# DIAGNijmegen/bodyct-dram-emph-subtype

Hardware: AMD Instinct MI355X
Metric: CT volumes/sec (train step, 1x128x256x256) (higher is better)
Workload: dtype f32; 1 GPU; BASELINE configs[1]: resnet18segcls train step (fwd+loss+bwd+Adam), batch 2/GPU, 1x128x256x256, fp32, inputs resident in HBM; global_batch=2, parallelism=dp1, hip_graph=False, streams=2

## Files before the change

### bodyct-dram-emph-subtype_amd/csrc/bn.hip

```cpp
#include <stdlib.h>
#include <atomic>
#include "common.h"

namespace {

template <typename T>
__global__ void reduce_partials_kernel(const T* __restrict__ partial, double* __restrict__ out, int nparts,
                                       int RC, double tail, int has_tail) {
  __shared__ double sm[256];
  const int col = blockIdx.x * 64 + (threadIdx.x & 63);
  const int lane4 = threadIdx.x >> 6;
  const int S = gridDim.y, sidx = blockIdx.y;
  double s = 0.0;
  if (col < RC)
    for (int p = sidx + S * lane4; p < nparts; p += 4 * S) s += (double)partial[(long)p * RC + col];
  sm[threadIdx.x] = s;
  __syncthreads();
  if (lane4 == 0 && col < RC)
    out[(long)sidx * RC + col] = sm[threadIdx.x] + sm[threadIdx.x + 64] + sm[threadIdx.x + 128] + sm[threadIdx.x + 192];
  if (has_tail && blockIdx.x == 0 && blockIdx.y == 0 && threadIdx.x == 0) out[RC] = tail;
}

__global__ void bn_finalize_kernel(const double* __restrict__ sums, double count_host,
                                   const double* __restrict__ count_dev, const float* __restrict__ gamma,
// ... 20 lines not shown
  }
  const double is = 1.0 / sqrt(v + (double)eps);
  const float sc = (float)((double)gamma[c] * is);
  mean[c] = (float)m;
  invstd[c] = (float)is;
  scale[c] = sc;
  shift[c] = (float)((double)beta[c] - m * (double)gamma[c] * is);
}

struct FoldFinalize {
  double count;
  const float* gamma; const float* beta; float* rmean; float* rvar;
  float momentum, eps; int update;
  float* mean; float* invstd; float* scale; float* shift;
};
constexpr int FOLD_XMAX = 512;

__global__ __launch_bounds__(1024) void fold_partials_kernel(const float* __restrict__ partial, double* scratch,
                                                             double* __restrict__ sums, float* __restrict__ sums_f32,
                                                             float* __restrict__ f32_row1, const int nparts, const int RC,
                                                             const double tail,
                                                             const int has_tail, unsigned* __restrict__ ticket,
                                                             const FoldFinalize ff) {
  __shared__ double sm[1024];
  __shared__ double tot[64];
  __shared__ unsigned s_ticket;
  const int t64 = threadIdx.x & 63, lane4 = threadIdx.x >> 6;
  const int C = RC >> 1;
  const int col = ff.gamma ? (t64 >> 5) * C + blockIdx.x * 32 + (t64 & 31) : blockIdx.x * 64 + t64;
  const bool live = ff.gamma ? (blockIdx.x * 32 + (t64 & 31) < C) : (col < RC);
  const int S = gridDim.y, sidx = blockIdx.y;
// ... 12 lines not shown
  }
  sm[threadIdx.x] = s;
  __syncthreads();
  double total = 0.0;
  if (lane4 == 0) {
#pragma unroll
    for (int j = 0; j < 16; ++j) total += sm[t64 + 64 * j];
  }
  if (S > 1) {
    if (lane4 == 0 && live) scratch[(long)sidx * RC + col] = total;
    __threadfence();
    __syncthreads();
    if (threadIdx.x == 0) s_ticket = atomicAdd(&ticket[blockIdx.x], 1u);
    __syncthreads();
    if (s_ticket != (unsigned)S - 1) return;
    __threadfence();
    if (lane4 == 0 && live) {
      total = 0.0;
      int k = 0;
      for (; k + 8 <= S; k += 8) {
        double v[8];
#pragma unroll
        for (int j = 0; j < 8; ++j)
          v[j] = __hip_atomic_load(scratch + (long)(k + j) * RC + col, __ATOMIC_RELAXED, __HIP_MEMORY_SCOPE_AGENT);
#pragma unroll
        for (int j = 0; j < 8; ++j) total += v[j];
      }
      for (; k < S; ++k)
        total += __hip_atomic_load(scratch + (long)k * RC + col, __ATOMIC_RELAXED, __HIP_MEMORY_SCOPE_AGENT);
    }
// ... 436 lines not shown
    DRAM_LAUNCH_CHECK();
    hipLaunchKernelGGL((reduce_partials_kernel<double>), dim3((RC + 63) / 64, 1), dim3(256), 0, st,
                       (const double*)scratch, sums, S, RC, tail, has_tail);
  }
  DRAM_LAUNCH_CHECK();
  return DRAM_OK;
}

extern "C" int dram_fold_partials_stages(int nparts) {
  if (nparts <= 1024) return 1;
  const int s = (nparts + 511) / 512;
  return s > 64 ? 64 : s;
}

static int fold_launch(const float* partial, double* sums, double* scratch, float* sums_f32, float* f32_row1, int nparts,
                       int RC, double tail, int has_tail, const FoldFinalize& ff, hipStream_t st) {
  const int S = dram_fold_partials_stages(nparts);
  const int gx = ff.gamma ? (RC / 2 + 31) / 32 : (RC + 63) / 64;
  if (S > 1 && gx > FOLD_XMAX) return DRAM_ERR_UNSUPPORTED;
  unsigned* ticket = nullptr;
  if (S > 1) {
    ticket = reinterpret_cast<unsigned*>(scratch + (long)S * RC);
    const hipError_t e = hipMemsetAsync(ticket, 0, sizeof(unsigned) * gx, st);
    if (e != hipSuccess) return (int)e;
  }
  DramProf prof(DRAM_FAM_BN, 0, 0.0, 4.0 * (double)nparts * RC + 8.0 * RC, st);
  hipLaunchKernelGGL(fold_partials_kernel, dim3(gx, S), dim3(1024), 0, st, partial, scratch, sums, sums_f32, f32_row1,
                     nparts, RC, tail, has_tail, ticket, ff);
  DRAM_LAUNCH_CHECK();
  return DRAM_OK;
}

extern "C" int dram_fold_partials(const float* partial, double* sums, double* scratch, float* sums_f32, float* f32_row1,
                                  int nparts, int R, int C, double tail, int has_tail, dram_stream_t stream) {
  if (!partial || !sums || !scratch || nparts < 1 || R < 1 || C < 1) return DRAM_ERR_BAD_ARG;
  if (f32_row1 && (R != 2 || !sums_f32)) return DRAM_ERR_BAD_ARG;
  FoldFinalize ff{};
  return fold_launch(partial, sums, scratch, sums_f32, f32_row1, nparts, R * C, tail, has_tail, ff, (hipStream_t)stream);
}

extern "C" int dram_bn_fold_finalize(const float* partial, double* sums, double* scratch, int nparts, int C, double count,
                                     const float* gamma, const float* beta, float* running_mean, float* running_var,
                                     float momentum, float eps, int update_running, float* mean, float* invstd,
                                     float* scale, float* shift, dram_stream_t stream) {
  if (!partial || !sums || !scratch || nparts < 1 || C < 1 || count <= 0.0) return DRAM_ERR_BAD_ARG;
  if (!gamma || !beta || !mean || !invstd || !scale || !shift) return DRAM_ERR_BAD_ARG;
  if (update_running && (!running_mean || !running_var)) return DRAM_ERR_BAD_ARG;
  FoldFinalize ff{count, gamma, beta, running_mean, running_var, momentum, eps, update_running, mean, invstd, scale, shift};
  return fold_launch(partial, sums, scratch, nullptr, nullptr, nparts, 2 * C, 0.0, 0, ff, (hipStream_t)stream);
}

extern "C" int dram_bn_finalize(const double* sums, double count, const double* count_dev, const float* gamma,
                                const float* beta,
                                float* running_mean, float* running_var, float momentum, float eps,
                                int update_running, float* mean, float* invstd, float* scale, float* shift, int C,
                                dram_stream_t stream) {
  if (!gamma || !beta || !mean || !invstd || !scale || !shift || C < 1) return DRAM_ERR_BAD_ARG;
  if (!sums && (!running_mean || !running_var)) return DRAM_ERR_BAD_ARG;
  if (sums && !count_dev && count <= 0.0) return DRAM_ERR_BAD_ARG;
  if (update_running && (!running_mean || !running_var)) return DRAM_ERR_BAD_ARG;
  DramProf prof(DRAM_FAM_BN, 1, 0.0, 4.0 * 10.0 * C, (hipStream_t)stream);
  hipLaunchKernelGGL(bn_finalize_kernel, dim3((C + 255) / 256), dim3(256), 0, (hipStream_t)stream, sums, count,
                     count_dev, gamma, beta, running_mean, running_var, momentum, eps, update_running, mean, invstd, scale,
                     shift, C);
// ... 189 lines not shown
```

### bodyct-dram-emph-subtype_amd/csrc/head_loss.hip

```cpp
#include "common.h"

namespace {

template <int NOT, typename T>
__global__ __launch_bounds__(256) void head_fwd_kernel(const T* __restrict__ x, const float* __restrict__ w,
                                                       const float* __restrict__ bias, const float* __restrict__ lungs,
                                                       NearGeom ng, float* __restrict__ dense,
                                                       float* __restrict__ partial, int D, int H, int W, int NO,
                                                       int sigmoid, int nblk) {
  __shared__ float wl[NOT * 32 + NOT];
  __shared__ float red[4][NOT + 1];
  const int tid = threadIdx.x;
  for (int i = tid; i < NO * 32; i += 256) wl[i] = w[i];
  for (int i = tid; i < NO; i += 256) wl[NOT * 32 + i] = bias[i];
  __syncthreads();
  const long b = blockIdx.y;
  const long vps = (long)D * H * W;
  float acc[NOT + 1];
#pragma unroll
  for (int c = 0; c <= NOT; ++c) acc[c] = 0.f;
  for (long v = blockIdx.x * 256L + tid; v < vps; v += (long)gridDim.x * 256L) {
    asm volatile("" ::: "memory");
    float4 xv[8];
#pragma unroll
// ... 401 lines not shown
      !pse_bands || n_cle < 1 || n_pse < 1 || B < 1 || !out || !coef || !greg)
    return DRAM_ERR_BAD_ARG;
  RegTail a;
  a.partial = partial; a.nblk = nblk;
  a.reg[0] = reg_cle; a.reg[1] = reg_pse;
  a.label[0] = cle_labels; a.label[1] = pse_labels;
  a.weight[0] = cle_w; a.weight[1] = pse_w;
  a.bands[0] = cle_bands; a.bands[1] = pse_bands;
  a.nband[0] = n_cle; a.nband[1] = n_pse;
  a.B = B; a.N = voxels_total; a.smooth = smooth; a.beta = beta; a.gamma = gamma;
  a.out = out; a.coef = coef; a.greg = greg;
  hipLaunchKernelGGL(regloss_tail_kernel, dim3(1), dim3(256), 0, (hipStream_t)stream, a);
  DRAM_LAUNCH_CHECK();
  return DRAM_OK;
}
```

### bodyct-dram-emph-subtype_amd/engine.py

```python
from __future__ import annotations

import os
import time
from typing import Dict, List, Optional

import torch

from . import ops
from .ops import ConvGeom

Tensor = torch.Tensor

ARCHS = {
    "resnet18": ("basic", (2, 2, 2, 2)),
    "resnet34": ("basic", (3, 4, 6, 3)),
    "resnet50": ("bottleneck", (3, 4, 6, 3)),
}
EXPANSION = {"basic": 1, "bottleneck": 4}
STAGES = ((64, 1, 1), (128, 2, 1), (256, 1, 2), (512, 1, 4))
BN_EPS = 1e-5
BN_MOMENTUM = 0.1


class _State:
# ... 70 lines not shown
        bnp = c["bn"]
        scale, shift = st.eval_ss[bnp]
        zmask = c["z"] if c.get("ss") is None else None
        if st.dist is not None:
            self._flush_wgrad(st)
        if st.need_param:
            part = ops.bn_bwd_reduce(dz, zmask, c["y"], c["mean"], c["invstd"], True, scale, shift)
            _, sf = ops.reduce_partials(part, want_f32=True)
            st.grads[bnp + ".weight"] = sf[1]
            st.grads[bnp + ".bias"] = sf[0]
        y = c["y"] if zmask is None else None
        if c.get("b") and st.need_param:
            dy, colpart = ops.bn_bwd_apply_eval(dz, zmask, y, scale, shift, True, want_colsum=True)
            if colpart is None:
                colpart = ops.colsum(dy)
            st.grads[c["b"]] = ops.reduce_partials(colpart)[0].float()
            return dy
        return ops.bn_bwd_apply_eval(dz, zmask, y, scale, shift, True)

    def _bn_bwd(self, st: _State, c: dict, dz: Tensor) -> Tensor:
        if not st.training:
            return self._bn_bwd_eval(st, c, dz)
        bnp = c["bn"]
        zmask, (sc, sh) = (c["z"], (None, None)) if c.get("ss") is None else (None, c["ss"])
        part = c.pop("part", None)
        if part is None:
            part = ops.bn_bwd_reduce(dz, zmask, c["y"], c["mean"], c["invstd"], True, sc, sh)
        sums, sf = ops.reduce_partials(part, want_f32=True)
        st.grads[bnp + ".weight"] = sf[1]
        st.grads[bnp + ".bias"] = sf[0]
        count, count_dev = c["count"]
        if st.dist is not None and st.dist.sync_bn:
            work = st.dist.all_reduce_stats_async(sums)
            self._flush_wgrad(st)
            work.wait()
        if c.get("b"):
            dy, colpart = ops.bn_bwd_apply(dz, zmask, c["y"], c["mean"], c["invstd"], st.P[bnp + ".weight"], sums,
                                           count, True, sc, sh, want_colsum=True, count_dev=count_dev)
            if colpart is None:
                colpart = ops.colsum(dy)
            st.grads[c["b"]] = ops.reduce_partials(colpart)[0].float()
            return dy
        return ops.bn_bwd_apply(dz, zmask, c["y"], c["mean"], c["invstd"], st.P[bnp + ".weight"], sums, count,
                                True, sc, sh, count_dev=count_dev)

    def _conv_bn_fwd(self, st: _State, x, wname: str, bname: Optional[str], bnp: str, k: int, stride: int,
                     pad: int, dil: int, residual=None, rs: int = 1, xr=None, defer_z: bool = False):
        w = st.P[wname]
        pro = None
        split = None
        if isinstance(x, tuple):
            split = x
            x = None
            B, D, H, W, _ = split[0].shape
            Cin = split[0].shape[4] + split[1].shape[4]
        elif isinstance(x, dict):
# ... 327 lines not shown
        for li, ((planes, stride, dil), nblk) in enumerate(zip(STAGES, self.layers)):
            for bi in range(nblk):
                s = stride if bi == 0 else 1
                has_ds = bi == 0 and (stride != 1 or inplanes != planes * self.e)
                h, c = self._block_fwd(st, h, f"layer{li + 1}.{bi}", planes, s, dil, has_ds)
                block_ctx.append(c)
                inplanes = planes * self.e
            feats.append(h)
        x1, x4f = feats[0], feats[3]
        xup1, cu1 = self._up_fwd(st, x4f, x1, "us1")
        xup2, cu2 = self._up_fwd(st, xup1, xs, "us2")
        xup3, cu3 = self._conv_bn_fwd(st, xup2, "us3.0.weight", "us3.0.bias", "us3.1", 3, 1, 1, 1)

        n0, n1 = P["fcs.0.weight"].shape[0], P["fcs.1.weight"].shape[0]
        NO = n0 + n1
        hw = torch.cat([P["fcs.0.weight"].reshape(n0, 32), P["fcs.1.weight"].reshape(n1, 32)], 0).contiguous()
        hb = torch.cat([P["fcs.0.bias"], P["fcs.1.bias"]], 0).contiguous()
        sig = self.head == "reg"
        dense, partial = ops.head_fwd(xup3, hw, hb, lungs4 if sig else None, sig)
        sums = partial.sum(1)
        denom = sums[:, NO]
        if sig:
            outs = [sums[:, 0] / denom, sums[:, 1] / denom]
        else:
            pooled = sums[:, :NO] / denom[:, None]
            outs = [pooled[:, :n0].contiguous(), pooled[:, n0:].contiguous()]
        dense_list = [dense[:, :n0], dense[:, n0:]]
        saved = None
        if need_grad:
            saved = dict(st=st, x4=x4, y0=y0, xs=xs, mean0=mean0, invstd0=invstd0, count0=count0, ss0=ss0, amax=amax,
                         blocks=block_ctx, cu1=cu1, cu2=cu2, cu3=cu3, xup3=xup3, hw=hw, dense=dense, lungs4=lungs4,
                         denom=denom, n0=n0, n1=n1, xs_shape=tuple(xs.shape))
        elif keep_head:
            saved = dict(xup3=xup3, hw=hw, hb=hb, dense=dense, lungs4=lungs4, denom=denom, n0=n0, n1=n1)
        if need_grad:
            self._conv_lists[shape_key] = list(st.convs)
            st.packed.clear()
        if st.nbt:
            torch._foreach_add_(st.nbt, 1)
        return dense_list, outs, saved

    def _head_cotangents(self, saved, g_dense, g_outs):
        n0, n1 = saved["n0"], saved["n1"]
        NO = n0 + n1
        dense = saved["dense"]
        B = dense.shape[0]
        sig = self.head == "reg"
        dev = dense.device
        gpool = torch.zeros((B, NO), device=dev, dtype=torch.float32)
        denom = saved["denom"]
        if sig:
            if g_outs[0] is not None:
                gpool[:, 0] = g_outs[0] / denom
            if g_outs[1] is not None:
                gpool[:, 1] = g_outs[1] / denom
        else:
            if g_outs[0] is not None:
                gpool[:, :n0] = g_outs[0] / denom[:, None]
            if g_outs[1] is not None:
                gpool[:, n0:] = g_outs[1] / denom[:, None]
        gd = None
        if g_dense[0] is not None or g_dense[1] is not None:
            gd = torch.zeros_like(dense)
            if g_dense[0] is not None:
                gd[:, :n0] = g_dense[0]
            if g_dense[1] is not None:
                gd[:, n0:] = g_dense[1]
        return gpool, gd

    def _backward(self, saved, g_dense, g_outs):
        st: _State = saved["st"]
        dist = st.dist if st.need_param else None
        if dist is not None:
            dist.begin_backward(saved["dense"].device)
        if st.need_param and self._two_streams():
            st.side = ops.side_stream(saved["dense"].device.index)

        n0, n1 = saved["n0"], saved["n1"]
        NO = n0 + n1
        dense = saved["dense"]
        sig = self.head == "reg"
        gpool, gd = self._head_cotangents(saved, g_dense, g_outs)
        dxup3, wpart = ops.head_bwd(saved["xup3"], saved["hw"], dense if sig else None, gd, gpool,
                                    saved["lungs4"] if sig else None, sig)
        if st.need_param:
            wg = ops.reduce_partials(wpart.reshape(wpart.shape[0], 1, NO * 33)).reshape(NO, 33).float()
            st.grads["fcs.0.weight"] = wg[:n0, :32].reshape(n0, 32, 1, 1, 1).contiguous()
            st.grads["fcs.0.bias"] = wg[:n0, 32].contiguous()
            st.grads["fcs.1.weight"] = wg[n0:, :32].reshape(n1, 32, 1, 1, 1).contiguous()
            st.grads["fcs.1.bias"] = wg[n0:, 32].contiguous()
        if dist is not None:
            dist.grads_ready(st.grads, ["fcs.0.weight", "fcs.0.bias", "fcs.1.weight", "fcs.1.bias"])

        dxup2 = self._conv_bn_bwd(st, saved["cu3"], dxup3, nxt=saved["cu2"][1])
        dxup1, dskip_stem = self._up_bwd(st, saved["cu2"], dxup2, skip_view=True)
        d, dskip_x1 = self._up_bwd(st, saved["cu1"], dxup1)

        blocks = saved["blocks"]
        idx = len(blocks)
        for li in (3, 2, 1, 0):
            nblk = self.layers[li]
            for bi in reversed(range(nblk)):
                idx -= 1
                extra = dskip_x1 if (li == 1 and bi == 0) else None
                d = self._block_bwd(st, blocks[idx], d, extra_add=extra)
# ... 39 lines not shown
```

### bodyct-dram-emph-subtype_amd/med3d.py

```python
from __future__ import annotations

if not __package__:
    import _dropin
    __package__ = _dropin.adopt(__name__)

import os
from typing import List, Optional

import torch
import torch.nn as nn

from . import ops
from .engine import ARCHS, EXPANSION, Engine

__all__ = ["ResNetSegCls", "ResNetSegReg", "resnet18segcls", "resnet34segcls", "resnet50segcls",
           "resnet18segreg", "resnet34segreg", "resnet50segreg", "BasicBlock", "Bottleneck",
           "UpsampleConvBlock5d"]


def _conv3(cin, cout, stride=1, dilation=1):
    return nn.Conv3d(cin, cout, kernel_size=3, dilation=dilation, stride=stride, padding=dilation, bias=False)


class _Container(nn.Module):
# ... 53 lines not shown
                                                    need_x=need_x, need_param=need_param)
        ctx.saved_state = saved
        ctx.module = module
        return dense[0], dense[1], outs[0], outs[1]

    @staticmethod
    def backward(ctx, gd0, gd1, go0, go1):
        module = ctx.module
        saved, ctx.saved_state = ctx.saved_state, None
        if saved is None:
            raise RuntimeError("backward through the Med3D engine a second time (buffers were freed)")

        def c(t):
            return None if t is None else t.contiguous()

        grads = module._engine.backward(saved, [c(gd0), c(gd1)], [c(go0), c(go1)])
        out = [None, saved.get("dx") if ctx.needs_input_grad[1] else None, None]
        for name, p in module._named_tensors()[0]:
            out.append(grads.get(name) if p.requires_grad else None)
        return tuple(out)


class _ResNetSeg(nn.Module):
    HEAD = None

    def __init__(self, block, layers, shortcut_type="A", n_classes=(6, 3)):
        super().__init__()
        if shortcut_type != "A":
            raise NotImplementedError("only shortcut_type='A' (every reference conf) is implemented")
        self.inplanes = 64
        self.conv1 = nn.Conv3d(1, 64, kernel_size=7, stride=(2, 2, 2), padding=(3, 3, 3), bias=False)
# ... 227 lines not shown
```

### bodyct-dram-emph-subtype_amd/models.py

```python
from __future__ import annotations

if not __package__:
    import _dropin
    __package__ = _dropin.adopt(__name__)

import os
from types import SimpleNamespace
from typing import Dict, List, Optional

import numpy as np
import torch
import torch.nn as nn
import torch.nn.functional as F

from . import ops
from .optim import FusedAdam
from .utils import get_model_by_name

try:
    import pytorch_lightning as pl
    _Base = pl.LightningModule
except Exception:
    pl = None

# ... 124 lines not shown
def reg_train_loss(dense_outs, reg_outs, lungs, ems, cle_labels, pse_labels, cle_w, pse_w):
    B = dense_outs[0].shape[0]

    def vol(t):
        return t.reshape(B, *t.shape[-3:]).float().contiguous()

    def row(t, dtype=torch.float32):
        return t.reshape(B).to(dtype).contiguous()

    loss, lc, lp, mul, seg = _RegLossFn.apply(vol(dense_outs[0]), vol(dense_outs[1]), vol(lungs), vol(ems),
                                              row(reg_outs[0]), row(reg_outs[1]), row(cle_labels, torch.int64),
                                              row(pse_labels, torch.int64), row(cle_w), row(pse_w))
    return loss, dict(loss_cle=lc, loss_pse=lp, mul_loss=mul, seg_loss=seg)


def cls_train_loss(cls_outs, cle_labels, pse_labels, cle_cw, pse_cw):
    loss_cle = F.cross_entropy(cls_outs[0], cle_labels, weight=cle_cw)
    loss_pse = F.cross_entropy(cls_outs[1], pse_labels, weight=pse_cw)
    return loss_cle + loss_pse, dict(loss_cle=loss_cle, loss_pse=loss_pse)


def update_class_weights(weights: torch.Tensor, y_true: torch.Tensor, y_pred: torch.Tensor) -> torch.Tensor:
    labels = torch.unique(torch.cat([y_true, y_pred]))
    if labels.numel() != weights.numel():
        raise ValueError(f"class-weight update: {labels.numel()} classes occur, {weights.numel()} weights "
                         "(the reference's element-wise product fails the same way)")
    hit = (y_true[None, :] == labels[:, None])
    acc = (hit & (y_pred[None, :] == labels[:, None])).sum(1).double() / hit.sum(1).double()
    w = weights.double().to(acc.device) * (1.0 - acc)
    return (w / w.sum()).to(weights.dtype).cpu()

# ... 339 lines not shown
```

### bodyct-dram-emph-subtype_amd/ops.py

```python
from __future__ import annotations

import contextlib
import ctypes
import functools
import math
import os
import threading
import weakref
from dataclasses import dataclass
from typing import Dict, List, Optional, Tuple

import torch

from . import _lib
from ._lib import DramConvDesc

Tensor = torch.Tensor


def _L():
    return _lib.load()


_TLS = threading.local()
# ... 780 lines not shown
    B, D, H, W = (int(v) for v in in_shape)
    if min(B, D, H, W) < 1:
        raise ValueError(f"stem_bwd_data: bad input shape {tuple(in_shape)}")
    sfx = _act(dy, "dy", (B, stem_out(D), stem_out(H), stem_out(W), 64))
    _req(w, "w", shape=(64, 1, 7, 7, 7))
    nbytes = _L().dram_stem_bwd_data_workspace(B, D, H, W)
    ws = torch.empty(((nbytes + 3) // 4,), device=dy.device, dtype=torch.float32)
    dx = torch.empty((B, D, H, W), device=dy.device, dtype=torch.float32)
    with _span("stem_dgrad_kernel+fold", 2.0 * dy.numel() * 343):
        _chk(_fn("dram_stem_bwd_data", sfx)(_p(dy), _p(w), _p(dx), B, D, H, W, _p(ws), nbytes, _stream()),
             "dram_stem_bwd_data" + sfx)
    return dx


FOLD_TICKET_DOUBLES = _lib.DRAM_FOLD_TICKET_DOUBLES


def reduce_partials(partial: Tensor, tail: Optional[float] = None, want_f32: bool = False):
    _req(partial, "partial")
    Pn, R, C = partial.shape
    stages = _L().dram_fold_partials_stages(Pn)
    n = R * C + (1 if tail is not None else 0)
    buf = torch.empty((n + stages * R * C + (FOLD_TICKET_DOUBLES if stages > 1 else 0),), device=partial.device,
                      dtype=torch.float64)
    flat = buf[:n]
    f32 = [torch.empty((C,), device=partial.device, dtype=torch.float32) for _ in range(R)] if want_f32 else None
    if want_f32 and R > 2:
        raise ValueError("reduce_partials: the float copy supports at most two rows")
    _chk(_L().dram_fold_partials(_p(partial), _p(flat), _p(buf[n:]), _p(f32[0]) if f32 else None,
                                 _p(f32[1]) if (f32 and R == 2) else None, Pn, R, C,
                                 float(tail) if tail is not None else 0.0, int(tail is not None), _stream()),
         "dram_fold_partials")
    res = (flat, flat[:R * C].view(R, C)) if tail is not None else (flat.view(R, C),)
    if want_f32:
        res = res + (f32,)
    return res if len(res) > 1 else res[0]


def bn_fold_finalize(partial: Tensor, count: float, gamma: Tensor, beta: Tensor, running_mean: Tensor,
                     running_var: Tensor, momentum: float, eps: float):
    _req(partial, "partial")
    Pn, R, C = partial.shape
    if R != 2:
        raise ValueError("bn_fold_finalize: expected [P,2,C] partial sums")
    for t, nm in ((gamma, "gamma"), (beta, "beta"), (running_mean, "running_mean"), (running_var, "running_var")):
        _req(t, nm, shape=(C,))
    stages = _L().dram_fold_partials_stages(Pn)
    buf = torch.empty(((1 + stages) * 2 * C + (FOLD_TICKET_DOUBLES if stages > 1 else 0),), device=partial.device,
                      dtype=torch.float64)
    out = torch.empty((4, C), device=partial.device, dtype=torch.float32)
    _chk(_L().dram_bn_fold_finalize(_p(partial), _p(buf), _p(buf[2 * C:]), Pn, C, float(count), _p(gamma), _p(beta),
                                    _p(running_mean), _p(running_var), float(momentum), float(eps), 1, _p(out[0]),
                                    _p(out[1]), _p(out[2]), _p(out[3]), _stream()), "dram_bn_fold_finalize")
    return out[0], out[1], out[2], out[3]


def bn_finalize(sums: Optional[Tensor], count: float, gamma: Tensor, beta: Tensor, running_mean: Tensor,
                running_var: Tensor, momentum: float, eps: float, update_running: bool,
                count_dev: Optional[Tensor] = None):
    C = gamma.numel()
    if count_dev is not None:
        _req(count_dev, "count_dev", dtype=torch.float64, shape=(1,))
    _req(gamma, "gamma", shape=(C,))
    _req(beta, "beta", shape=(C,))
    _req(running_mean, "running_mean", shape=(C,))
    _req(running_var, "running_var", shape=(C,))
    if sums is not None:
        _req(sums, "sums", dtype=torch.float64, shape=(2, C))
# ... 719 lines not shown
        _req(dense, "dense", shape=(B, NO, D, H, W))
    if gdense is not None:
        _req(gdense, "gdense", shape=(B, NO, D, H, W))
    Dl = Hl = Wl = 0
    if lungs is not None:
        _req(lungs, "lungs")
        _, Dl, Hl, Wl = lungs.shape
    nparts = _L().dram_head_bwd_nparts(D * H * W)
    dx = torch.empty_like(x)
    wpartial = torch.empty((B * nparts, NO, 33), device=x.device, dtype=torch.float32)
    _chk(_fn("dram_head_bwd", sfx)(_p(x), _p(w), _p(dense), _p(gdense), _p(gpool), _p(lungs), Dl, Hl, Wl, _p(dx),
                                   _p(wpartial), B, D, H, W, NO, int(sigmoid), _stream()), "dram_head_bwd")
    return dx, wpartial


CAM_METHODS = {"gradcam": _lib.DRAM_CAM_GRADCAM, "hirescam": _lib.DRAM_CAM_HIRESCAM, "layercam": _lib.DRAM_CAM_LAYERCAM}


def cam(x: Tensor, w: Tensor, bias: Tensor, gdense: Optional[Tensor], gpool: Tensor, lungs: Optional[Tensor],
        sigmoid: bool, method: str = "gradcam", relu: bool = True) -> Tensor:
    if method not in CAM_METHODS:
        raise ValueError(f"cam: unknown method {method!r} (one of {sorted(CAM_METHODS)})")
    sfx = _act(x, "x")
    if x.dim() != 5 or x.shape[-1] != 32:
        raise ValueError("cam: x must be the 32-channel us3 output [B,D,H,W,32]")
    B, D, H, W, _ = x.shape
    if min(B, D, H, W) < 1 or x.numel() >= 2 ** 31:
        raise ValueError("cam: x must be non-empty and hold fewer than 2^31 elements")
    NO = w.shape[0]
    _req(w, "w", shape=(NO, 32))
# ... 202 lines not shown
```

### include/dram_hip.h

```cpp
#ifndef DRAM_HIP_H
#define DRAM_HIP_H

#include <stddef.h>
#include <stdint.h>

#ifdef __cplusplus
extern "C" {
#endif

typedef void* dram_stream_t;

#define DRAM_OK 0
#define DRAM_ERR_BAD_ARG (-1)
#define DRAM_ERR_UNSUPPORTED (-2)
#define DRAM_ERR_WORKSPACE (-3)

#define DRAM_ABI_VERSION 7
int dram_version(void);
const char* dram_build_info(void);
const char* dram_abi_hash(void);
unsigned long long dram_stream_capture_id(dram_stream_t stream);

enum {
  DRAM_FAM_CONV_WINO2D = 0,
// ... 113 lines not shown

int dram_conv_algo(const DramConvDesc* desc);

int dram_stem_num_tiles(int B, int Do, int Ho, int Wo);
int dram_stem_fwd(const float* x, const float* w, float* y, float* stats_partial, int B, int D, int H,
                  int W, dram_stream_t stream);
size_t dram_stem_bwd_weight_workspace(int B, int D, int H, int W);
int dram_stem_bwd_weight(const float* x, const float* dy, float* dw, int B, int D, int H, int W,
                         void* workspace, size_t workspace_bytes, dram_stream_t stream);
size_t dram_stem_bwd_data_workspace(int B, int D, int H, int W);
int dram_stem_bwd_data(const float* dy, const float* w, float* dx, int B, int D, int H, int W, void* workspace,
                       size_t workspace_bytes, dram_stream_t stream);

int dram_reduce_partials_stages(int nparts);
#define DRAM_FOLD_TICKET_DOUBLES 256
int dram_fold_partials_stages(int nparts);
int dram_fold_partials(const float* partial, double* sums, double* scratch, float* sums_f32, float* f32_row1, int nparts,
                       int R, int C, double tail, int has_tail, dram_stream_t stream);
int dram_bn_fold_finalize(const float* partial, double* sums, double* scratch, int nparts, int C, double count,
                          const float* gamma, const float* beta, float* running_mean, float* running_var, float momentum,
                          float eps, int update_running, float* mean, float* invstd, float* scale, float* shift,
                          dram_stream_t stream);
int dram_reduce_partials(const float* partial, double* sums, double* scratch, int nparts, int R, int C,
                         double tail, int has_tail, dram_stream_t stream);

int dram_bn_finalize(const double* sums, double count, const double* count_dev, const float* gamma, const float* beta,
                     float* running_mean, float* running_var, float momentum, float eps,
                     int update_running, float* mean, float* invstd, float* scale, float* shift,
                     int C, dram_stream_t stream);

int dram_bn_apply(const float* y, const float* scale, const float* shift, const float* residual,
                  int Dr, int Hr, int Wr, int Cr, int rs, float* z, int B, int D, int H, int W, int C,
                  int relu, dram_stream_t stream);

int dram_colsum_nparts(long long rows, int C);
int dram_bn_bwd_reduce(const float* dz, const float* z, const float* y, const float* mean,
                       const float* invstd, const float* scale, const float* shift, float* partial,
// ... 25 lines not shown
int dram_upmix_axis_fwd_final(const float* in, const void* base, void* out, int out_bf16, float* stats, long long outer,
                              int Ni, int m, int C, dram_stream_t stream);
int dram_upmix_axis_bwd(const void* g, int g_bf16, void* h, int h_bf16, long long outer, int Ni, int m, int C,
                        dram_stream_t stream);
int dram_upmix_split_weight(const float* w, float* wlo, float* ws, int Co, int Cu, int Cs, dram_stream_t stream);
int dram_upmix_merge_wgrad(const float* dwlo, const float* dws, float* dw, int Co, int Cu, int Cs, dram_stream_t stream);

int dram_head_nblk(long long voxels_per_sample);
int dram_head_fwd(const float* x, const float* w, const float* bias, const float* lungs, int Dl, int Hl,
                  int Wl, float* dense, float* partial, int B, int D, int H, int W, int NO, int sigmoid,
                  dram_stream_t stream);
int dram_head_bwd_nparts(long long voxels_per_sample);
int dram_head_bwd(const float* x, const float* w, const float* dense, const float* gdense,
                  const float* gpool, const float* lungs, int Dl, int Hl, int Wl, float* dx,
                  float* wpartial, int B, int D, int H, int W, int NO, int sigmoid, dram_stream_t stream);

#define DRAM_CAM_GRADCAM 0
#define DRAM_CAM_HIRESCAM 1
#define DRAM_CAM_LAYERCAM 2
int dram_cam_nblk(long long voxels_per_sample);
int dram_cam_point(const float* x, const float* w, const float* bias, const float* gdense, const float* gpool,
                   const float* lungs, int Dl, int Hl, int Wl, float* out, int B, int D, int H, int W, int NO,
                   int sigmoid, int method, int relu, dram_stream_t stream);
int dram_cam_sum(const float* x, const float* w, const float* bias, const float* gdense, const float* gpool,
                 const float* lungs, int Dl, int Hl, int Wl, float* partial, int B, int D, int H, int W, int NO,
                 int sigmoid, dram_stream_t stream);
int dram_cam_combine(const float* x, const float* w, const double* sums, float* out, int B, int D, int H, int W,
                     int NO, int relu, dram_stream_t stream);

int dram_segloss_nblk(long long voxels_total);
// ... 231 lines not shown
```

Baseline: 55.73 volumes/sec.

## Fuse head and classification-loss glue ops into single kernels and reuse fold tickets

Replaces many small torch ops in the classifier head (weight concat, score division, gpool scatter, weight-grad slicing, cross-entropy tail) with single-block custom kernels. It also adds persistent self-resetting tickets for the multi-stage fold kernel, so the per-call hipMemsetAsync is skipped. Bias grads now come from the f32 output of the reduction instead of a separate cast. The goal is fewer launches and less host dispatch per train step, at the cost of extra custom-kernel code with single-block serial loops.

```diff
diff --git a/bodyct-dram-emph-subtype_amd/csrc/bn.hip b/bodyct-dram-emph-subtype_amd/csrc/bn.hip
--- a/bodyct-dram-emph-subtype_amd/csrc/bn.hip
+++ b/bodyct-dram-emph-subtype_amd/csrc/bn.hip
@@ -58,7 +58,8 @@
   float momentum, eps; int update;
   float* mean; float* invstd; float* scale; float* shift;
 };
-constexpr int FOLD_XMAX = 512;
+constexpr int FOLD_XMAX = DRAM_FOLD_TICKET_WORDS;
+static_assert(FOLD_XMAX * sizeof(unsigned) <= DRAM_FOLD_TICKET_DOUBLES * sizeof(double), "per-call ticket words fit");
 
 __global__ __launch_bounds__(1024) void fold_partials_kernel(const float* __restrict__ partial, double* scratch,
                                                              double* __restrict__ sums, float* __restrict__ sums_f32,
@@ -101,6 +102,7 @@
     if (threadIdx.x == 0) s_ticket = atomicAdd(&ticket[blockIdx.x], 1u);
     __syncthreads();
     if (s_ticket != (unsigned)S - 1) return;
+    if (threadIdx.x == 0) __hip_atomic_store(&ticket[blockIdx.x], 0u, __ATOMIC_RELAXED, __HIP_MEMORY_SCOPE_AGENT);
     __threadfence();
     if (lane4 == 0 && live) {
       total = 0.0;
@@ -567,12 +569,12 @@
 }
 
 static int fold_launch(const float* partial, double* sums, double* scratch, float* sums_f32, float* f32_row1, int nparts,
-                       int RC, double tail, int has_tail, const FoldFinalize& ff, hipStream_t st) {
+                       int RC, double tail, int has_tail, const FoldFinalize& ff, void* tickets, hipStream_t st) {
   const int S = dram_fold_partials_stages(nparts);
   const int gx = ff.gamma ? (RC / 2 + 31) / 32 : (RC + 63) / 64;
   if (S > 1 && gx > FOLD_XMAX) return DRAM_ERR_UNSUPPORTED;
-  unsigned* ticket = nullptr;
-  if (S > 1) {
+  unsigned* ticket = static_cast<unsigned*>(tickets);
+  if (S > 1 && !ticket) {
     ticket = reinterpret_cast<unsigned*>(scratch + (long)S * RC);
     const hipError_t e = hipMemsetAsync(ticket, 0, sizeof(unsigned) * gx, st);
     if (e != hipSuccess) return (int)e;
@@ -585,22 +587,24 @@
 }
 
 extern "C" int dram_fold_partials(const float* partial, double* sums, double* scratch, float* sums_f32, float* f32_row1,
-                                  int nparts, int R, int C, double tail, int has_tail, dram_stream_t stream) {
+                                  int nparts, int R, int C, double tail, int has_tail, void* tickets,
+                                  dram_stream_t stream) {
   if (!partial || !sums || !scratch || nparts < 1 || R < 1 || C < 1) return DRAM_ERR_BAD_ARG;
   if (f32_row1 && (R != 2 || !sums_f32)) return DRAM_ERR_BAD_ARG;
   FoldFinalize ff{};
-  return fold_launch(partial, sums, scratch, sums_f32, f32_row1, nparts, R * C, tail, has_tail, ff, (hipStream_t)stream);
+  return fold_launch(partial, sums, scratch, sums_f32, f32_row1, nparts, R * C, tail, has_tail, ff, tickets,
+                     (hipStream_t)stream);
 }
 
 extern "C" int dram_bn_fold_finalize(const float* partial, double* sums, double* scratch, int nparts, int C, double count,
                                      const float* gamma, const float* beta, float* running_mean, float* running_var,
                                      float momentum, float eps, int update_running, float* mean, float* invstd,
-                                     float* scale, float* shift, dram_stream_t stream) {
+                                     float* scale, float* shift, void* tickets, dram_stream_t stream) {
   if (!partial || !sums || !scratch || nparts < 1 || C < 1 || count <= 0.0) return DRAM_ERR_BAD_ARG;
   if (!gamma || !beta || !mean || !invstd || !scale || !shift) return DRAM_ERR_BAD_ARG;
   if (update_running && (!running_mean || !running_var)) return DRAM_ERR_BAD_ARG;
   FoldFinalize ff{count, gamma, beta, running_mean, running_var, momentum, eps, update_running, mean, invstd, scale, shift};
-  return fold_launch(partial, sums, scratch, nullptr, nullptr, nparts, 2 * C, 0.0, 0, ff, (hipStream_t)stream);
+  return fold_launch(partial, sums, scratch, nullptr, nullptr, nparts, 2 * C, 0.0, 0, ff, tickets, (hipStream_t)stream);
 }
 
 extern "C" int dram_bn_finalize(const double* sums, double count, const double* count_dev, const float* gamma,
diff --git a/bodyct-dram-emph-subtype_amd/csrc/head_loss.hip b/bodyct-dram-emph-subtype_amd/csrc/head_loss.hip
--- a/bodyct-dram-emph-subtype_amd/csrc/head_loss.hip
+++ b/bodyct-dram-emph-subtype_amd/csrc/head_loss.hip
@@ -439,3 +439,173 @@
   DRAM_LAUNCH_CHECK();
   return DRAM_OK;
 }
+
+namespace {
+
+__global__ __launch_bounds__(256) void head_pack_kernel(const float* __restrict__ w0, const float* __restrict__ b0,
+                                                        int n0, const float* __restrict__ w1,
+                                                        const float* __restrict__ b1, int n1, float* __restrict__ hw,
+                                                        float* __restrict__ hb) {
+  const int NO = n0 + n1;
+  for (int i = threadIdx.x; i < NO * 32; i += 256) hw[i] = i < n0 * 32 ? w0[i] : w1[i - n0 * 32];
+  for (int i = threadIdx.x; i < NO; i += 256) hb[i] = i < n0 ? b0[i] : b1[i - n0];
+}
+
+__global__ __launch_bounds__(256) void head_scores_kernel(const float* __restrict__ sums, int B, int n0, int n1,
+                                                          float* __restrict__ out0, float* __restrict__ out1) {
+  const int NO = n0 + n1;
+  for (int i = threadIdx.x; i < B * NO; i += 256) {
+    const int b = i / NO, c = i - b * NO;
+    const float v = sums[(long)b * (NO + 1) + c] / sums[(long)b * (NO + 1) + NO];
+    if (c < n0) out0[(long)b * n0 + c] = v;
+    else out1[(long)b * n1 + (c - n0)] = v;
+  }
+}
+
+__global__ __launch_bounds__(256) void head_gpool_kernel(const float* __restrict__ g0, long long s0,
+                                                         const float* __restrict__ g1, long long s1,
+                                                         const float* __restrict__ denom, long long sd, int B, int n0,
+                                                         int n1, float* __restrict__ gpool) {
+  const int NO = n0 + n1;
+  for (int i = threadIdx.x; i < B * NO; i += 256) {
+    const int b = i / NO, c = i - b * NO;
+    const float* g = c < n0 ? g0 : g1;
+    const long long off = c < n0 ? b * s0 + c : b * s1 + (c - n0);
+    gpool[i] = g ? g[off] / denom[b * sd] : 0.f;
+  }
+}
+
+__global__ __launch_bounds__(256) void head_wgrad_split_kernel(const double* __restrict__ sums, int n0, int n1,
+                                                               float* __restrict__ w0, float* __restrict__ b0,
+                                                               float* __restrict__ w1, float* __restrict__ b1) {
+  const int NO = n0 + n1;
+  for (int i = threadIdx.x; i < NO * 33; i += 256) {
+    const int c = i / 33, k = i - c * 33;
+    const float v = (float)sums[i];
+    if (c < n0) {
+      if (k < 32) w0[c * 32 + k] = v;
+      else b0[c] = v;
+    } else {
+      if (k < 32) w1[(c - n0) * 32 + k] = v;
+      else b1[c - n0] = v;
+    }
+  }
+}
+
+struct ClsTail {
+  const float* x[2]; const long long* y[2]; const float* w[2]; int n[2];
+  int B;
+  float* out;
+  float* g;
+};
+
+__device__ inline double cls_lse(const float* x, int n) {
+  double m = (double)x[0];
+  for (int c = 1; c < n; ++c) m = fmax(m, (double)x[c]);
+  double s = 0.0;
+  for (int c = 0; c < n; ++c) s += exp((double)x[c] - m);
+  return m + log(s);
+}
+
+__global__ __launch_bounds__(256) void cls_loss_tail_kernel(ClsTail a) {
+  __shared__ double red[2][256];
+  __shared__ double tot[2][2];
+  const int tid = threadIdx.x;
+  const int NO = a.n[0] + a.n[1];
+  for (int h = 0; h < 2; ++h) {
+    const int n = a.n[h];
+    double num = 0.0, den = 0.0;
+    for (int b = tid; b < a.B; b += 256) {
+      const long long lab = a.y[h][b];
+      if (lab == -100) continue;
+      if (lab < 0 || lab >= n) { num = nan(""); continue; }
+      const float* x = a.x[h] + (long)b * n;
+      const double w = (double)a.w[h][lab];
+      num += w * (cls_lse(x, n) - (double)x[lab]);
+      den += w;
+    }
+    red[0][tid] = num; red[1][tid] = den;
+    __syncthreads();
+    for (int s = 128; s > 0; s >>= 1) {
+      if (tid < s) { red[0][tid] += red[0][tid + s]; red[1][tid] += red[1][tid + s]; }
+      __syncthreads();
+    }
+    if (tid == 0) { tot[h][0] = red[0][0]; tot[h][1] = red[1][0]; }
+    __syncthreads();
+  }
+  for (int h = 0; h < 2; ++h) {
+    const int n = a.n[h], c0 = h ? a.n[0] : 0;
+    const double den = tot[h][1];
+    const bool poisoned = tot[h][0] != tot[h][0];
+    for (int b = tid; b < a.B; b += 256) {
+      const long long lab = a.y[h][b];
+      float* g = a.g + (long)b * NO + c0;
+      if (lab < 0 || lab >= n) {
+        for (int c = 0; c < n; ++c) g[c] = (poisoned && lab != -100) ? nanf("") : 0.f;
+        continue;
+      }
+      const float* x = a.x[h] + (long)b * n;
+      const double lse = cls_lse(x, n), k = (double)a.w[h][lab] / den;
+      for (int c = 0; c < n; ++c) g[c] = (float)(k * (exp((double)x[c] - lse) - (c == lab ? 1.0 : 0.0)));
+    }
+  }
+  if (tid == 0) {
+    const float l0 = (float)(tot[0][0] / tot[0][1]), l1 = (float)(tot[1][0] / tot[1][1]);
+    a.out[0] = l0 + l1; a.out[1] = l0; a.out[2] = l1;
+  }
+}
+
+inline bool head_counts_ok(int n0, int n1) { return n0 >= 1 && n1 >= 1 && n0 + n1 <= 16; }
+
+}
+
+extern "C" int dram_head_pack(const float* w0, const float* b0, int n0, const float* w1, const float* b1, int n1,
+                              float* hw, float* hb, dram_stream_t stream) {
+  if (!w0 || !b0 || !w1 || !b1 || !hw || !hb || !head_counts_ok(n0, n1)) return DRAM_ERR_BAD_ARG;
+  hipLaunchKernelGGL(head_pack_kernel, dim3(1), dim3(256), 0, (hipStream_t)stream, w0, b0, n0, w1, b1, n1, hw, hb);
+  DRAM_LAUNCH_CHECK();
+  return DRAM_OK;
+}
+
+extern "C" int dram_head_scores(const float* sums, int B, int n0, int n1, float* out0, float* out1,
+                                dram_stream_t stream) {
+  if (!sums || !out0 || !out1 || B < 1 || !head_counts_ok(n0, n1)) return DRAM_ERR_BAD_ARG;
+  if ((long long)B * (n0 + n1 + 1) >= (1LL << 31)) return DRAM_ERR_UNSUPPORTED;
+  hipLaunchKernelGGL(head_scores_kernel, dim3(1), dim3(256), 0, (hipStream_t)stream, sums, B, n0, n1, out0, out1);
+  DRAM_LAUNCH_CHECK();
+  return DRAM_OK;
+}
+
+extern "C" int dram_head_gpool(const float* g0, long long stride0, const float* g1, long long stride1,
+                               const float* denom, long long denom_stride, int B, int n0, int n1, float* gpool,
+                               dram_stream_t stream) {
+  if (!denom || !gpool || B < 1 || !head_counts_ok(n0, n1) || stride0 < 0 || stride1 < 0 || denom_stride < 0)
+    return DRAM_ERR_BAD_ARG;
+  if ((long long)B * (n0 + n1) >= (1LL << 31)) return DRAM_ERR_UNSUPPORTED;
+  hipLaunchKernelGGL(head_gpool_kernel, dim3(1), dim3(256), 0, (hipStream_t)stream, g0, stride0, g1, stride1, denom,
+                     denom_stride, B, n0, n1, gpool);
+  DRAM_LAUNCH_CHECK();
+  return DRAM_OK;
+}
+
+extern "C" int dram_head_wgrad_split(const double* sums, int n0, int n1, float* w0, float* b0, float* w1, float* b1,
+                                     dram_stream_t stream) {
+  if (!sums || !w0 || !b0 || !w1 || !b1 || !head_counts_ok(n0, n1)) return DRAM_ERR_BAD_ARG;
+  hipLaunchKernelGGL(head_wgrad_split_kernel, dim3(1), dim3(256), 0, (hipStream_t)stream, sums, n0, n1, w0, b0, w1, b1);
+  DRAM_LAUNCH_CHECK();
+  return DRAM_OK;
+}
+
+extern "C" int dram_cls_loss_tail(const float* x0, const float* x1, const long long* y0, const long long* y1,
+                                  const float* w0, const float* w1, int B, int n0, int n1, float* out, float* gouts,
+                                  dram_stream_t stream) {
+  if (!x0 || !x1 || !y0 || !y1 || !w0 || !w1 || !out || !gouts || B < 1 || !head_counts_ok(n0, n1))
+    return DRAM_ERR_BAD_ARG;
+  if ((long long)B * (n0 + n1) >= (1LL << 31)) return DRAM_ERR_UNSUPPORTED;
+  ClsTail a;
+  a.x[0] = x0; a.x[1] = x1; a.y[0] = y0; a.y[1] = y1; a.w[0] = w0; a.w[1] = w1; a.n[0] = n0; a.n[1] = n1;
+  a.B = B; a.out = out; a.g = gouts;
+  hipLaunchKernelGGL(cls_loss_tail_kernel, dim3(1), dim3(256), 0, (hipStream_t)stream, a);
+  DRAM_LAUNCH_CHECK();
+  return DRAM_OK;
+}
diff --git a/bodyct-dram-emph-subtype_amd/engine.py b/bodyct-dram-emph-subtype_amd/engine.py
--- a/bodyct-dram-emph-subtype_amd/engine.py
+++ b/bodyct-dram-emph-subtype_amd/engine.py
@@ -108,7 +108,7 @@
             dy, colpart = ops.bn_bwd_apply_eval(dz, zmask, y, scale, shift, True, want_colsum=True)
             if colpart is None:
                 colpart = ops.colsum(dy)
-            st.grads[c["b"]] = ops.reduce_partials(colpart)[0].float()
+            st.grads[c["b"]] = ops.reduce_partials(colpart, want_f32=True)[1][0]
             return dy
         return ops.bn_bwd_apply_eval(dz, zmask, y, scale, shift, True)
 
@@ -133,7 +133,7 @@
                                            count, True, sc, sh, want_colsum=True, count_dev=count_dev)
             if colpart is None:
                 colpart = ops.colsum(dy)
-            st.grads[c["b"]] = ops.reduce_partials(colpart)[0].float()
+            st.grads[c["b"]] = ops.reduce_partials(colpart, want_f32=True)[1][0]
             return dy
         return ops.bn_bwd_apply(dz, zmask, c["y"], c["mean"], c["invstd"], st.P[bnp + ".weight"], sums, count,
                                 True, sc, sh, count_dev=count_dev)
@@ -491,17 +491,13 @@
 
         n0, n1 = P["fcs.0.weight"].shape[0], P["fcs.1.weight"].shape[0]
         NO = n0 + n1
-        hw = torch.cat([P["fcs.0.weight"].reshape(n0, 32), P["fcs.1.weight"].reshape(n1, 32)], 0).contiguous()
-        hb = torch.cat([P["fcs.0.bias"], P["fcs.1.bias"]], 0).contiguous()
+        hw, hb = ops.head_pack(P["fcs.0.weight"], P["fcs.0.bias"], P["fcs.1.weight"], P["fcs.1.bias"])
         sig = self.head == "reg"
         dense, partial = ops.head_fwd(xup3, hw, hb, lungs4 if sig else None, sig)
         sums = partial.sum(1)
         denom = sums[:, NO]
-        if sig:
-            outs = [sums[:, 0] / denom, sums[:, 1] / denom]
-        else:
-            pooled = sums[:, :NO] / denom[:, None]
-            outs = [pooled[:, :n0].contiguous(), pooled[:, n0:].contiguous()]
+        o0, o1 = ops.head_scores(sums, n0, n1)
+        outs = [o0.reshape(B), o1.reshape(B)] if sig else [o0, o1]
         dense_list = [dense[:, :n0], dense[:, n0:]]
         saved = None
         if need_grad:
@@ -519,23 +515,8 @@
 
     def _head_cotangents(self, saved, g_dense, g_outs):
         n0, n1 = saved["n0"], saved["n1"]
-        NO = n0 + n1
         dense = saved["dense"]
-        B = dense.shape[0]
-        sig = self.head == "reg"
-        dev = dense.device
-        gpool = torch.zeros((B, NO), device=dev, dtype=torch.float32)
-        denom = saved["denom"]
-        if sig:
-            if g_outs[0] is not None:
-                gpool[:, 0] = g_outs[0] / denom
-            if g_outs[1] is not None:
-                gpool[:, 1] = g_outs[1] / denom
-        else:
-            if g_outs[0] is not None:
-                gpool[:, :n0] = g_outs[0] / denom[:, None]
-            if g_outs[1] is not None:
-                gpool[:, n0:] = g_outs[1] / denom[:, None]
+        gpool = ops.head_gpool(g_outs[0], g_outs[1], saved["denom"], n0, n1)
         gd = None
         if g_dense[0] is not None or g_dense[1] is not None:
             gd = torch.zeros_like(dense)
@@ -561,11 +542,9 @@
         dxup3, wpart = ops.head_bwd(saved["xup3"], saved["hw"], dense if sig else None, gd, gpool,
                                     saved["lungs4"] if sig else None, sig)
         if st.need_param:
-            wg = ops.reduce_partials(wpart.reshape(wpart.shape[0], 1, NO * 33)).reshape(NO, 33).float()
-            st.grads["fcs.0.weight"] = wg[:n0, :32].reshape(n0, 32, 1, 1, 1).contiguous()
-            st.grads["fcs.0.bias"] = wg[:n0, 32].contiguous()
-            st.grads["fcs.1.weight"] = wg[n0:, :32].reshape(n1, 32, 1, 1, 1).contiguous()
-            st.grads["fcs.1.bias"] = wg[n0:, 32].contiguous()
+            wg = ops.reduce_partials(wpart.reshape(wpart.shape[0], 1, NO * 33)).reshape(NO, 33)
+            (st.grads["fcs.0.weight"], st.grads["fcs.0.bias"], st.grads["fcs.1.weight"],
+             st.grads["fcs.1.bias"]) = ops.head_wgrad_split(wg, n0, n1)
         if dist is not None:
             dist.grads_ready(st.grads, ["fcs.0.weight", "fcs.0.bias", "fcs.1.weight", "fcs.1.bias"])
 
diff --git a/bodyct-dram-emph-subtype_amd/med3d.py b/bodyct-dram-emph-subtype_amd/med3d.py
--- a/bodyct-dram-emph-subtype_amd/med3d.py
+++ b/bodyct-dram-emph-subtype_amd/med3d.py
@@ -91,7 +91,7 @@
         def c(t):
             return None if t is None else t.contiguous()
 
-        grads = module._engine.backward(saved, [c(gd0), c(gd1)], [c(go0), c(go1)])
+        grads = module._engine.backward(saved, [c(gd0), c(gd1)], [go0, go1])
         out = [None, saved.get("dx") if ctx.needs_input_grad[1] else None, None]
         for name, p in module._named_tensors()[0]:
             out.append(grads.get(name) if p.requires_grad else None)
diff --git a/bodyct-dram-emph-subtype_amd/models.py b/bodyct-dram-emph-subtype_amd/models.py
--- a/bodyct-dram-emph-subtype_amd/models.py
+++ b/bodyct-dram-emph-subtype_amd/models.py
@@ -162,7 +162,51 @@
     return loss, dict(loss_cle=lc, loss_pse=lp, mul_loss=mul, seg_loss=seg)
 
 
+class _ClsLossFn(torch.autograd.Function):
+
+    @staticmethod
+    def forward(ctx, o0, o1, cle_labels, pse_labels, cle_cw, pse_cw):
+        ctx.set_materialize_grads(False)
+        with ops.launch_scope(o0.device):
+            out, gouts = ops.cls_loss_tail(o0, o1, cle_labels, pse_labels, cle_cw, pse_cw)
+        ctx.save_for_backward(gouts)
+        ctx.n0 = o0.shape[1]
+        loss, lc, lp = out.unbind(0)
+        ctx.mark_non_differentiable(lc, lp)
+        return loss, lc, lp
+
+    @staticmethod
+    @torch.autograd.function.once_differentiable
+    def backward(ctx, g, *_):
+        if g is None:
+            return None, None, None, None, None, None
+        (gouts,) = ctx.saved_tensors
+        gs = gouts * g
+        return gs[:, :ctx.n0], gs[:, ctx.n0:], None, None, None, None
+
+
+def _cls_tail_ok(cls_outs, cle_labels, pse_labels, cle_cw, pse_cw) -> bool:
+    o0, o1 = cls_outs[0], cls_outs[1]
+    if not all(isinstance(t, torch.Tensor) for t in (o0, o1, cle_labels, pse_labels, cle_cw, pse_cw)):
+        return False
+    if o0.dim() != 2 or o1.dim() != 2 or o0.shape[0] != o1.shape[0] or o0.shape[0] < 1:
+        return False
+    B, n0, n1 = o0.shape[0], o0.shape[1], o1.shape[1]
+    if n0 < 1 or n1 < 1 or n0 + n1 > 16:
+        return False
+    for t, dtype, shape in ((o0, torch.float32, (B, n0)), (o1, torch.float32, (B, n1)),
+                            (cle_labels, torch.int64, (B,)), (pse_labels, torch.int64, (B,)),
+                            (cle_cw, torch.float32, (n0,)), (pse_cw, torch.float32, (n1,))):
+        if not t.is_cuda or t.device != o0.device or t.dtype != dtype or tuple(t.shape) != shape:
+            return False
+    return not (cle_labels.requires_grad or cle_cw.requires_grad or pse_cw.requires_grad)
+
+
 def cls_train_loss(cls_outs, cle_labels, pse_labels, cle_cw, pse_cw):
+    if _cls_tail_ok(cls_outs, cle_labels, pse_labels, cle_cw, pse_cw):
+        loss, lc, lp = _ClsLossFn.apply(cls_outs[0].contiguous(), cls_outs[1].contiguous(), cle_labels.contiguous(),
+                                        pse_labels.contiguous(), cle_cw.contiguous(), pse_cw.contiguous())
+        return loss, dict(loss_cle=lc, loss_pse=lp)
     loss_cle = F.cross_entropy(cls_outs[0], cle_labels, weight=cle_cw)
     loss_pse = F.cross_entropy(cls_outs[1], pse_labels, weight=pse_cw)
     return loss_cle + loss_pse, dict(loss_cle=loss_cle, loss_pse=loss_pse)
diff --git a/bodyct-dram-emph-subtype_amd/ops.py b/bodyct-dram-emph-subtype_amd/ops.py
--- a/bodyct-dram-emph-subtype_amd/ops.py
+++ b/bodyct-dram-emph-subtype_amd/ops.py
@@ -818,6 +818,37 @@
 
 
 FOLD_TICKET_DOUBLES = _lib.DRAM_FOLD_TICKET_DOUBLES
+FOLD_TICKET_WORDS = _lib.DRAM_FOLD_TICKET_WORDS
+_TICKET_SETS = 256
+_TICKET_POOL: Dict[int, Tensor] = {}
+_TICKET_SLOT: Dict[tuple, int] = {}
+_TICKET_LOCK = threading.Lock()
+FOLD_TICKETS_PERSISTENT = True
+
+
+def fold_tickets(stages: int = 2) -> Optional[Tensor]:
+    if stages <= 1 or not FOLD_TICKETS_PERSISTENT:
+        return None
+    dev = _launch_device()
+    cid = capture_id()
+    key = (dev, _stream().value, cid)
+    with _TICKET_LOCK:
+        pool = _TICKET_POOL.get(dev)
+        if pool is None:
+            if cid:
+                return None
+            pool = torch.zeros((_TICKET_SETS, FOLD_TICKET_WORDS), device=torch.device("cuda", dev), dtype=torch.int32)
+            done = torch.cuda.Event()
+            done.record()
+            done.synchronize()
+            _TICKET_POOL[dev] = pool
+        slot = _TICKET_SLOT.get(key)
+        if slot is None:
+            slot = sum(1 for k in _TICKET_SLOT if k[0] == dev)
+            if slot >= _TICKET_SETS:
+                return None
+            _TICKET_SLOT[key] = slot
+    return pool[slot]
 
 
 def reduce_partials(partial: Tensor, tail: Optional[float] = None, want_f32: bool = False):
@@ -825,15 +856,17 @@
     Pn, R, C = partial.shape
     stages = _L().dram_fold_partials_stages(Pn)
     n = R * C + (1 if tail is not None else 0)
-    buf = torch.empty((n + stages * R * C + (FOLD_TICKET_DOUBLES if stages > 1 else 0),), device=partial.device,
-                      dtype=torch.float64)
+    tickets = fold_tickets(stages)
+    buf = torch.empty((n + stages * R * C + (FOLD_TICKET_DOUBLES if stages > 1 and tickets is None else 0),),
+                      device=partial.device, dtype=torch.float64)
     flat = buf[:n]
     f32 = [torch.empty((C,), device=partial.device, dtype=torch.float32) for _ in range(R)] if want_f32 else None
     if want_f32 and R > 2:
         raise ValueError("reduce_partials: the float copy supports at most two rows")
     _chk(_L().dram_fold_partials(_p(partial), _p(flat), _p(buf[n:]), _p(f32[0]) if f32 else None,
                                  _p(f32[1]) if (f32 and R == 2) else None, Pn, R, C,
-                                 float(tail) if tail is not None else 0.0, int(tail is not None), _stream()),
+                                 float(tail) if tail is not None else 0.0, int(tail is not None), _p(tickets),
+                                 _stream()),
          "dram_fold_partials")
     res = (flat, flat[:R * C].view(R, C)) if tail is not None else (flat.view(R, C),)
     if want_f32:
@@ -850,12 +883,14 @@
     for t, nm in ((gamma, "gamma"), (beta, "beta"), (running_mean, "running_mean"), (running_var, "running_var")):
         _req(t, nm, shape=(C,))
     stages = _L().dram_fold_partials_stages(Pn)
-    buf = torch.empty(((1 + stages) * 2 * C + (FOLD_TICKET_DOUBLES if stages > 1 else 0),), device=partial.device,
-                      dtype=torch.float64)
+    tickets = fold_tickets(stages)
+    buf = torch.empty(((1 + stages) * 2 * C + (FOLD_TICKET_DOUBLES if stages > 1 and tickets is None else 0),),
+                      device=partial.device, dtype=torch.float64)
     out = torch.empty((4, C), device=partial.device, dtype=torch.float32)
     _chk(_L().dram_bn_fold_finalize(_p(partial), _p(buf), _p(buf[2 * C:]), Pn, C, float(count), _p(gamma), _p(beta),
                                     _p(running_mean), _p(running_var), float(momentum), float(eps), 1, _p(out[0]),
-                                    _p(out[1]), _p(out[2]), _p(out[3]), _stream()), "dram_bn_fold_finalize")
+                                    _p(out[1]), _p(out[2]), _p(out[3]), _p(tickets), _stream()),
+         "dram_bn_fold_finalize")
     return out[0], out[1], out[2], out[3]
 
 
@@ -1605,6 +1640,92 @@
     return dx, wpartial
 
 
+def head_pack(w0: Tensor, b0: Tensor, w1: Tensor, b1: Tensor):
+    n0, n1 = w0.shape[0], w1.shape[0]
+    if n0 < 1 or n1 < 1 or n0 + n1 > 16:
+        raise ValueError("head_pack: 1 <= n0, n1 and n0 + n1 <= 16")
+    for t, nm, n in ((w0, "w0", n0), (w1, "w1", n1)):
+        _req(t, nm)
+        if t.numel() != n * 32:
+            raise ValueError(f"head_pack: {nm} must hold [n,32] weights")
+    _req(b0, "b0", shape=(n0,))
+    _req(b1, "b1", shape=(n1,))
+    hw = torch.empty((n0 + n1, 32), device=w0.device, dtype=torch.float32)
+    hb = torch.empty((n0 + n1,), device=w0.device, dtype=torch.float32)
+    _chk(_L().dram_head_pack(_p(w0), _p(b0), n0, _p(w1), _p(b1), n1, _p(hw), _p(hb), _stream()), "dram_head_pack")
+    return hw, hb
+
+
+def head_scores(sums: Tensor, n0: int, n1: int):
+    B = sums.shape[0]
+    _req(sums, "sums", shape=(B, n0 + n1 + 1))
+    if B < 1 or n0 < 1 or n1 < 1 or n0 + n1 > 16:
+        raise ValueError("head_scores: B >= 1, 1 <= n0, n1 and n0 + n1 <= 16")
+    out0 = torch.empty((B, n0), device=sums.device, dtype=torch.float32)
+    out1 = torch.empty((B, n1), device=sums.device, dtype=torch.float32)
+    _chk(_L().dram_head_scores(_p(sums), B, n0, n1, _p(out0), _p(out1), _stream()), "dram_head_scores")
+    return out0, out1
+
+
+def head_gpool(g0: Optional[Tensor], g1: Optional[Tensor], denom: Tensor, n0: int, n1: int) -> Tensor:
+    if denom.dim() != 1 or denom.dtype != torch.float32 or not denom.is_cuda or denom.device.index != _launch_device():
+        raise ValueError("head_gpool: denom must be a float32 [B] tensor on the launch device")
+    B = denom.shape[0]
+    if B < 1 or n0 < 1 or n1 < 1 or n0 + n1 > 16:
+        raise ValueError("head_gpool: B >= 1, 1 <= n0, n1 and n0 + n1 <= 16")
+    gs, strides = [], []
+    for g, n, nm in ((g0, n0, "g0"), (g1, n1, "g1")):
+        if g is not None:
+            if not isinstance(g, Tensor) or not g.is_cuda or g.device.index != _launch_device():
+                raise RuntimeError(f"head_gpool: {nm} must live on the launch device")
+            if tuple(g.shape) not in ((B, n),) + (((B,),) if n == 1 else ()):
+                raise ValueError(f"head_gpool: {nm} must be [B,{n}], got {tuple(g.shape)}")
+            if g.dtype != torch.float32:
+                g = g.float()
+            if (g.dim() == 2 and n > 1 and g.stride(1) != 1) or g.stride(0) < 0:
+                g = g.contiguous()
+        gs.append(g)
+        strides.append(0 if g is None else g.stride(0))
+    gpool = torch.empty((B, n0 + n1), device=denom.device, dtype=torch.float32)
+    _chk(_L().dram_head_gpool(_p(gs[0]), strides[0], _p(gs[1]), strides[1], _p(denom), denom.stride(0), B, n0, n1,
+                              _p(gpool), _stream()), "dram_head_gpool")
+    return gpool
+
+
+def head_wgrad_split(sums: Tensor, n0: int, n1: int):
+    _req(sums, "sums", dtype=torch.float64, shape=(n0 + n1, 33))
+    if n0 < 1 or n1 < 1 or n0 + n1 > 16:
+        raise ValueError("head_wgrad_split: 1 <= n0, n1 and n0 + n1 <= 16")
+    dev = sums.device
+    w0 = torch.empty((n0, 32, 1, 1, 1), device=dev, dtype=torch.float32)
+    b0 = torch.empty((n0,), device=dev, dtype=torch.float32)
+    w1 = torch.empty((n1, 32, 1, 1, 1), device=dev, dtype=torch.float32)
+    b1 = torch.empty((n1,), device=dev, dtype=torch.float32)
+    _chk(_L().dram_head_wgrad_split(_p(sums), n0, n1, _p(w0), _p(b0), _p(w1), _p(b1), _stream()),
+         "dram_head_wgrad_split")
+    return w0, b0, w1, b1
+
+
+def cls_loss_tail(x0: Tensor, x1: Tensor, y0: Tensor, y1: Tensor, w0: Tensor, w1: Tensor):
+    if x0.dim() != 2 or x1.dim() != 2:
+        raise ValueError("cls_loss_tail: logits must be [B,n0] and [B,n1]")
+    B, n0 = x0.shape
+    n1 = x1.shape[1]
+    _req(x0, "x0")
+    _req(x1, "x1", shape=(B, n1))
+    if B < 1 or n0 < 1 or n1 < 1 or n0 + n1 > 16:
+        raise ValueError("cls_loss_tail: B >= 1, 1 <= n0, n1 and n0 + n1 <= 16")
+    _req(y0, "y0", dtype=torch.int64, shape=(B,))
+    _req(y1, "y1", dtype=torch.int64, shape=(B,))
+    _req(w0, "w0", shape=(n0,))
+    _req(w1, "w1", shape=(n1,))
+    out = torch.empty(3, device=x0.device, dtype=torch.float32)
+    gouts = torch.empty((B, n0 + n1), device=x0.device, dtype=torch.float32)
+    _chk(_L().dram_cls_loss_tail(_p(x0), _p(x1), _p(y0), _p(y1), _p(w0), _p(w1), B, n0, n1, _p(out), _p(gouts),
+                                 _stream()), "dram_cls_loss_tail")
+    return out, gouts
+
+
 CAM_METHODS = {"gradcam": _lib.DRAM_CAM_GRADCAM, "hirescam": _lib.DRAM_CAM_HIRESCAM, "layercam": _lib.DRAM_CAM_LAYERCAM}
 
 
diff --git a/include/dram_hip.h b/include/dram_hip.h
--- a/include/dram_hip.h
+++ b/include/dram_hip.h
@@ -151,13 +151,14 @@
 
 int dram_reduce_partials_stages(int nparts);
 #define DRAM_FOLD_TICKET_DOUBLES 256
+#define DRAM_FOLD_TICKET_WORDS 512
 int dram_fold_partials_stages(int nparts);
 int dram_fold_partials(const float* partial, double* sums, double* scratch, float* sums_f32, float* f32_row1, int nparts,
-                       int R, int C, double tail, int has_tail, dram_stream_t stream);
+                       int R, int C, double tail, int has_tail, void* tickets, dram_stream_t stream);
 int dram_bn_fold_finalize(const float* partial, double* sums, double* scratch, int nparts, int C, double count,
                           const float* gamma, const float* beta, float* running_mean, float* running_var, float momentum,
                           float eps, int update_running, float* mean, float* invstd, float* scale, float* shift,
-                          dram_stream_t stream);
+                          void* tickets, dram_stream_t stream);
 int dram_reduce_partials(const float* partial, double* sums, double* scratch, int nparts, int R, int C,
                          double tail, int has_tail, dram_stream_t stream);
 
@@ -213,6 +214,17 @@
 int dram_head_bwd(const float* x, const float* w, const float* dense, const float* gdense,
                   const float* gpool, const float* lungs, int Dl, int Hl, int Wl, float* dx,
                   float* wpartial, int B, int D, int H, int W, int NO, int sigmoid, dram_stream_t stream);
+
+int dram_head_pack(const float* w0, const float* b0, int n0, const float* w1, const float* b1, int n1, float* hw,
+                   float* hb, dram_stream_t stream);
+int dram_head_scores(const float* sums, int B, int n0, int n1, float* out0, float* out1, dram_stream_t stream);
+int dram_head_gpool(const float* g0, long long stride0, const float* g1, long long stride1, const float* denom,
+                    long long denom_stride, int B, int n0, int n1, float* gpool, dram_stream_t stream);
+int dram_head_wgrad_split(const double* sums, int n0, int n1, float* w0, float* b0, float* w1, float* b1,
+                          dram_stream_t stream);
+
+int dram_cls_loss_tail(const float* x0, const float* x1, const long long* y0, const long long* y1, const float* w0,
+                       const float* w1, int B, int n0, int n1, float* out, float* gouts, dram_stream_t stream);
 
 #define DRAM_CAM_GRADCAM 0
 #define DRAM_CAM_HIRESCAM 1
```

Result: no change. 55.54 volumes/sec (-0.4%).
